# llehouerou/go-mp3

Hardware: AMD Instinct MI355X
Metric: MP3 frames/sec (44.1 kHz stereo 128 kbps) at 1/2/4/8 GPUs; max |ΔPCM| LSB (higher is better)
Workload: dtype f32; 1 GPU; c3: 1,024 independently seeded streams x 1,024 frames, 44.1 kHz stereo 128 kbps CBR (synthetic Layer III writer, seeds 1..1024); streams_per_gpu=1024, mode=fast (+-1 LSB vs reference), parallelism=1 independent ranks (stream sharding, no data-path collective), granules_per_gpu=2097152, chunks=16384, halo_granules=30720

## Files before the change

go-mp3_amd/csrc/granule_fast.hip:

```cpp
#pragma clang fp contract(fast)
#include <type_traits>

#include "dct32.h"
#include "dct4_18.h"
#include "xlane.h"

namespace mp3g {
namespace v3 {
#ifndef MP3G_FAST_PRIO
#define MP3G_FAST_PRIO 1
#endif
#ifndef MP3G_FAST_WG_WAVES
#define MP3G_FAST_WG_WAVES 8
#endif
constexpr int kWaves = MP3G_FAST_WG_WAVES;
namespace {

using common::hdr_combo;
using common::hdr_mode;
using common::hdr_nch;
__device__ __forceinline__ int pcm_sample(float sum) {
  return (int)__builtin_amdgcn_fmed3f(sum * 32767.0f, -32767.0f, 32767.0f);
}

constexpr int kLanes = 64;
using pk::f2;
__device__ __forceinline__ f2 pfma(f2 a, f2 b, f2 c) { return __builtin_elementwise_fma(a, b, c); }
__device__ __forceinline__ f2 bcast(float v) { return (f2){v, v}; }
__device__ __forceinline__ int kPretab(int sfb) { return (int)((0x2fe95400000ull >> (2 * sfb)) & 3u); }
constexpr int kHist = 16;
#ifndef MP3G_FAST_WAVES_PER_SIMD
#define MP3G_FAST_WAVES_PER_SIMD 4
#endif
constexpr int kSlots = kHist + 18;
static_assert(kSlots == kFastRingSlots, "FastTables::sinfo indexes the staged ring");
#ifndef MP3G_FAST_DWIN_STRIDE
#define MP3G_FAST_DWIN_STRIDE 20
#endif
constexpr int kDwinStride = MP3G_FAST_DWIN_STRIDE;

struct __align__(16) SharedSmem {
  float4 winp[4][2][9];
  float isr[8][2];
  float dwin[32][kDwinStride];
  uint2 lbd[kCombos][32];
  __device__ uint32_t lband_at(int c, int k) const { return lbd[c][k].x; }
  float p43[kFastP43];
};
struct __align__(16) WaveSmem {
  float ring[2][32][kSlots];
  mp3g_granule desc;
  _Float16 expo[2 * 22 + 2 * 39];
  __device__ float* expo_gain() { return reinterpret_cast<float*>(expo); }
  __device__ const float* expo_gain() const { return reinterpret_cast<const float*>(expo); }
  uint32_t zone[8][2];
};
constexpr uint32_t kZones = 8;
static_assert(kZones <= kZoneListPerChunk, "zone list smaller than a chunk's zones");

__device__ __forceinline__ void load_lines(const int16_t* coef, uint32_t g, int lane, uint32_t cw[9],
                                           int nbytes = (int)(MP3G_COEF_PER_GRANULE * sizeof(int16_t))) {
  const __amdgpu_buffer_rsrc_t rc = __builtin_amdgcn_make_buffer_rsrc(
      const_cast<int16_t*>(coef + (size_t)g * MP3G_COEF_PER_GRANULE), (short)0, nbytes,
      0x00020000);
  const int off = (lane >> 5) * 1152 + (lane & 31) * 36;
#pragma unroll
  for (int i = 0; i < 3; i++) {
    const auto v = __builtin_amdgcn_raw_buffer_load_b96(rc, off + 12 * i, 0, 0);
    cw[3 * i] = v[0];
    cw[3 * i + 1] = v[1];
    cw[3 * i + 2] = v[2];
  }
}

__device__ __forceinline__ void load_lines_lim(const int16_t* coef, uint32_t g, int lane, uint32_t cw[9], int nbytes,
                                               int lim) {
  const __amdgpu_buffer_rsrc_t rc = __builtin_amdgcn_make_buffer_rsrc(
      const_cast<int16_t*>(coef + (size_t)g * MP3G_COEF_PER_GRANULE), (short)0, nbytes,
      0x00020000);
  const int l0 = 18 * (lane & 31);
  const int off = (lane >> 5) * 1152 + 2 * l0;
#pragma unroll
  for (int i = 0; i < 3; i++) {
    const auto v = __builtin_amdgcn_raw_buffer_load_b96(rc, l0 + 6 * i < lim ? off + 12 * i : kNoRecord, 0, 0);
    cw[3 * i] = v[0];
    cw[3 * i + 1] = v[1];
    cw[3 * i + 2] = v[2];
  }
}
__device__ __forceinline__ uint32_t load_desc_dword(const mp3g_granule* gran, uint32_t g, int lane, bool valid) {
  const __amdgpu_buffer_rsrc_t rd = __builtin_amdgcn_make_buffer_rsrc(
      const_cast<mp3g_granule*>(gran + g), (short)0, valid ? (int)sizeof(mp3g_granule) : 0, 0x00020000);
  return __builtin_amdgcn_raw_buffer_load_b32(rd, 4 * lane, 0, 0);
}
__device__ __forceinline__ uint32_t desc_word(uint32_t dv, int k) {
  return (uint32_t)__builtin_amdgcn_readlane((int)dv, k);
}
__device__ __forceinline__ uint32_t desc_byte(uint32_t dv, int b) {
  return ((uint32_t)__builtin_amdgcn_ds_bpermute((b >> 2) << 2, (int)dv) >> (8 * (b & 3))) & 0xffu;
}
static_assert(sizeof(mp3g_granule) == 160 && offsetof(mp3g_granule, ch) == 8 && sizeof(mp3g_channel) == 72 &&
                  offsetof(mp3g_channel, scalefac_l) == 11,
              "descriptor dword layout");

__device__ __forceinline__ int count1_lim(const mp3g_granule* gran, uint32_t g, int lane) {
  const uint32_t h = gran[g].header;
  const int c0 = gran[g].ch[0].count1, c1 = gran[g].ch[1].count1;
  return (lane >> 5) ? (common::hdr_nch(h) == 2 ? c1 : 0) : c0;
}

__device__ void prologue(const ChunkDesc& cd, const mp3g_granule* gran, uint64_t* w_out, int init_in[2],
                         int lane) {
  const uint64_t c0 = cd.out_first, s0 = cd.stream_first;
  const bool have_in = cd.flags & kChunkStateIn;
  if (c0 == s0) {
    *w_out = c0;
    init_in[0] = init_in[1] = have_in;
    return;
  }
  const uint64_t start0 = (c0 >= 2 && c0 - 2 > s0) ? c0 - 2 : s0;
  const bool st1 = hdr_nch(gran[c0 - 1].header) == 2;
  const bool st2 = (c0 >= 2 && c0 - 2 >= s0) ? hdr_nch(gran[c0 - 2].header) == 2 : false;
  if (st1 && st2) {
    *w_out = start0;
    init_in[0] = init_in[1] = (start0 == s0) && have_in;
    return;
  }
  int any = 0;
  for (uint32_t k = lane; k < cd.n_out; k += kLanes) any |= hdr_nch(gran[c0 + k].header) == 2;
  const bool need1 = __ballot(any) != 0 || (cd.flags & kChunkStateOut);
  uint64_t start1 = c0;
  bool ch1_from_in = false;
  if (need1) {
    int found = 0;
    uint64_t p2 = 0;
    for (uint64_t hi = c0; hi > s0 && found < 2;) {
      const uint64_t lo = hi - s0 > kLanes ? hi - kLanes : s0;
      const uint64_t g = hi - 1 - lane;
      const bool stereo = ((uint64_t)lane < hi - lo) && hdr_nch(gran[g].header) == 2;
      uint64_t m = __ballot(stereo);
      while (m && found < 2) {
        const int b = __ffsll((unsigned long long)m) - 1;
        found++;
        if (found == 2) p2 = hi - 1 - b;
        m &= m - 1;
      }
      hi = lo;
    }
    if (found == 2) start1 = p2;
    else if (found == 1) start1 = s0;
    else ch1_from_in = true;
  }
  const uint64_t w = start0 < start1 ? start0 : start1;
  *w_out = w;
  init_in[0] = (w == s0) && have_in;
  init_in[1] = ch1_from_in ? have_in : ((w == s0) && have_in);
}

__device__ __forceinline__ void wave_sync() {
  __builtin_amdgcn_fence(__ATOMIC_RELEASE, "wavefront");
  __builtin_amdgcn_wave_barrier();
  __builtin_amdgcn_fence(__ATOMIC_ACQUIRE, "wavefront");
}

__device__ __forceinline__ void settle_vmem() { __builtin_amdgcn_s_waitcnt(0x0f70); }

__device__ __forceinline__ float self(bool c, float a, float b) {
  const int m = -(int)c;
  return __int_as_float((__float_as_int(a) & m) | (__float_as_int(b) & ~m));
}
__device__ __forceinline__ int seli(bool c, int a, int b) {
  const int m = -(int)c;
  return (a & m) | (b & ~m);
}

__device__ __forceinline__ float requant_fast(int xi, _Float16 e) {
  const float xf = (float)xi;
  const float t = __builtin_fmaf(__builtin_amdgcn_logf(fabsf(xf)), 1.0f / 3.0f, (float)e);
  return xf * __builtin_amdgcn_exp2f(t);
}

__device__ __forceinline__ float requant_gain(uint32_t xw, float g) {
  const float xf = (float)(int16_t)xw;
  return xf * __builtin_amdgcn_exp2f(__builtin_amdgcn_logf(fabsf(xf)) * (1.0f / 3.0f)) * g;
}

__device__ __forceinline__ float x_from_v(const float* v, int m) { return m >= 16 ? v[m - 16] : -v[48 - m]; }
template <int kS = kSlots>
__device__ __forceinline__ float v_from_x(const float* x, int i) {
  if (i < 16) return x[kS * dct32::kPosOfM[16 + i]];
  if (i == 16) return 0.0f;
  if (i < 48) return -x[kS * dct32::kPosOfM[48 - i]];
  return -x[kS * dct32::kPosOfM[i - 48]];
}

#ifndef MP3G_HOT_S
#define MP3G_HOT_S 4.0f
#endif
constexpr float kHotS = MP3G_HOT_S;
#ifndef MP3G_HOT_CHECK
#define MP3G_HOT_CHECK 1
#endif
#ifndef MP3G_HOT_L1
#define MP3G_HOT_L1 64.0f
#endif
constexpr float kHotL1 = MP3G_HOT_L1;

__device__ __forceinline__ float rmul(float a, float b) {
#pragma clang fp contract(off)
  return a * b;
}
__device__ __forceinline__ float radd(float a, float b) {
#pragma clang fp contract(off)
  return a + b;
}
__device__ __forceinline__ float rsub(float a, float b) {
#pragma clang fp contract(off)
  return a - b;
}

__device__ __forceinline__ float requant_exact(int xi, _Float16 e) {
  const int n4 = (int)((float)e * 4.0f);
  const float v = __builtin_ldexpf(g_req[n4 & 3][min(abs(xi), 8206)], n4 >> 2);
  return xi < 0 ? -v : v;
}

__device__ __forceinline__ const float* vtab(const float* p) {
  asm volatile("" : "+s"(p));
  return p;
}
typedef const float __attribute__((address_space(4))) cfloat4;
__device__ __forceinline__ cfloat4* stab(const float* p) {
  cfloat4* q = (cfloat4*)p;
  asm volatile("" : "+s"(q));
  return q;
}

template <int kS = kSlots>
__device__ __forceinline__ bool slot_sums_hot(const float (&ring)[2][32][kS], int nch, int cur = kHist) {
  const int lane = lane_fresh();
  const int c = lane >> 5, slot = lane & 31;
  float sum = 0.0f;
  if (c < nch && slot < 18) {
#pragma unroll
    for (int sb = 0; sb < 32; sb++) sum += fabsf(ring[c][sb][cur + slot]);
  }
  return __builtin_amdgcn_ballot_w64(sum > kHotL1) != 0;
}

__device__ __forceinline__ float max_abs18(const float* v) {
  float m = 0.0f;
#pragma unroll
  for (int j = 0; j < 18; j++) m = fmaxf(m, fabsf(v[j]));
  return m;
}

__device__ __forceinline__ void imdct_exact(const float x[18], int bt, int k, bool act, f2 stp[9], float o[18]) {
#pragma clang fp contract(off)
  const float sodd = (k & 1) ? -1.0f : 1.0f;
  const float* c12 = vtab(&g_fast.cos12[0][0]);
  const float* c36 = vtab(&g_fast.c36[0][0]);
  const float* win = vtab(&g_fast.win[0][0]) + 36 * bt;
  float st[18];
#pragma unroll
  for (int q = 0; q < 9; q++) {
    st[q] = stp[q].x;
    st[17 - q] = stp[q].y;
  }
  if (bt == 2) {
#pragma unroll
    for (int pos = 0; pos < 36; pos++) {
      float raw = 0.0f;
#pragma unroll
      for (int wi = 0; wi < 3; wi++) {
        const int p = pos - 6 - 6 * wi;
        if (p < 0 || p >= 12) continue;
        float sum = 0.0f;
#pragma unroll
        for (int m = 0; m < 6; m++) sum = sum + x[wi + 3 * m] * c12[12 * m + p];
        raw = raw + sum * win[p];
      }
      const float f = (pos & 1) ? raw * sodd : raw;
      if (pos < 18) o[pos] = f + st[pos];
      else if (act) st[pos - 18] = f;
    }
  } else {
    float d[18];
#pragma unroll
    for (int q = 0; q < 18; q++) {
      float s = 0.0f;
#pragma unroll
      for (int m = 0; m < 18; m++) s = s + x[m] * c36[18 * m + q];
      d[q] = s;
    }
#pragma unroll
    for (int pos = 0; pos < 36; pos++) {
      const float v = pos < 9 ? d[pos] : pos < 18 ? -d[17 - pos] : pos < 27 ? d[pos - 9] : d[44 - pos];
      const float raw = v * win[pos];
      const float f = (pos & 1) ? raw * sodd : raw;
      if (pos < 18) o[pos] = f + st[pos];
      else if (act) st[pos - 18] = f;
    }
  }
#pragma unroll
  for (int q = 0; q < 9; q++) stp[q] = (f2){st[q], st[17 - q]};
}

template <int kS = kSlots>
__device__ __forceinline__ void matrix_exact(float* colu) {
#pragma clang fp contract(off)
  float S[32];
#pragma unroll
  for (int j = 0; j < 32; j++) S[j] = colu[kS * j];
  for (int m = 0; m < 32; m++) {
    const float* row = vtab(&g_fast.nrow[m][0]);
    float s = 0.0f;
#pragma unroll
    for (int j = 0; j < 32; j++) s = s + row[j] * S[j];
    colu[kS * dct32::kPosOfM[m]] = s;
  }
}

template <int cur = kHist>
__device__ __forceinline__ void window_exact(const float* RA, const float* RB, int k, f2 acc2[9]) {
#pragma clang fp contract(off)
  float dw[16];
#pragma unroll
  for (int j = 0; j < 16; j++) dw[j] = vtab(&g_fast.dwin[0][0])[16 * k + j];
#pragma unroll
  for (int ss = 0; ss < 18; ss++) {
    float sum = 0.0f;
#pragma unroll
    for (int j = 0; j < 16; j++) sum = sum + ((j & 1) ? RB : RA)[cur + ss - j] * dw[j];
    const float t = sum * 32767.0f;
    if (ss & 1) acc2[ss >> 1].y = t;
    else acc2[ss >> 1].x = t;
  }
}
// ... 161 lines not shown
    } else {
      const __amdgpu_buffer_rsrc_t rl = __builtin_amdgcn_make_buffer_rsrc(
          const_cast<uint32_t*>(&g_fast.linfo[P.combo][0]), (short)0, 576 * 4, 0x00020000);
#pragma unroll
      for (int j = 0; j < 18; j++) {
        const uint32_t info = __builtin_amdgcn_raw_buffer_load_b32(rl, 4 * (18 * k0 + j), 0, 0);
        const int sfl = info & 31, sfs = (info >> 5) & 15, wown = (info >> 11) & 3;
        const bool lp = mixed0 && sfl < 8 && sfl >= nl_is;
        const bool sp = sfs < 12 && (!mixed0 || sfs >= 3) && sfs >= ns_is;
        const int pl = lp ? min((int)C0.scalefac_l[min(sfl, 21)], 7) : 7;
        const int ps = sp ? min((int)C0.scalefac_s[min(sfs, 12)][min(wown, 2)], 7) : 7;
        x[j] = x[j] * sh.isr[pl][ch] * sh.isr[ps][ch];
      }
    }
  }
}

template <bool kExact>
__device__ __forceinline__ void antialias_stage(float x[18], const GranParams& P, bool act, int k) {
  const bool sw = P.shortblk;
  const bool skip = !act || (sw && !P.mixed);
  const int sblim = (sw && P.mixed) ? 2 : 32;
  const bool lower = !skip && k >= 1 && k < sblim;
  const bool upper = !skip && k < 31 && k + 1 < sblim;
  float up[8], dn[8];
#pragma unroll
  for (int i = 0; i < 8; i++) {
    up[i] = xl::from_prev(x[17 - i]);
    dn[i] = xl::from_next(x[i]);
  }
#pragma unroll
  for (int i = 0; i < 8; i++) {
    const float cs = g_fast.aa_cs[i], ca = g_fast.aa_ca[i];
    const float ui = x[i], li = x[17 - i];
    if (kExact) {
      x[i] = self(lower, radd(rmul(ui, cs), rmul(up[i], ca)), ui);
      x[17 - i] = self(upper, rsub(rmul(li, cs), rmul(dn[i], ca)), li);
    } else {
      x[i] = self(lower, ui * cs + up[i] * ca, ui);
      x[17 - i] = self(upper, li * cs - dn[i] * ca, li);
    }
  }
}

__device__ __forceinline__ int imdct_block_type(uint32_t d1, int k) {
  int bt = (int)((d1 >> 16) & 3u);
  if ((d1 & 0xff00ff00u) == 0x01000100u && k < 2) bt = 0;
  return bt;
}

__device__ __forceinline__ void imdct_fast(const float x[18], int bt, int nch, bool act, float sodd,
                                           const SharedSmem& sh, f2 stp[9], float o[18]) {
  if (bt == 2) {
    float st[18];
#pragma unroll
    for (int q = 0; q < 9; q++) {
      st[q] = stp[q].x;
      st[17 - q] = stp[q].y;
    }
#pragma unroll
    for (int pos = 0; pos < 36; pos++) {
      float raw = 0.0f;
#pragma unroll
      for (int wi = 0; wi < 3; wi++) {
        const int p = pos - 6 - 6 * wi;
        if (p < 0 || p >= 12) continue;
        float sum = 0.0f;
#pragma unroll
        for (int m = 0; m < 6; m++) sum += x[wi + 3 * m] * dct4::kCos12[p][m];
        raw += sum * dct4::kWin12[p];
      }
      if (pos & 1) raw *= sodd;
      if (pos < 18) o[pos] = raw + st[pos];
      else st[pos - 18] = self(act, raw, st[pos - 18]);
    }
#pragma unroll
    for (int q = 0; q < 9; q++) stp[q] = (f2){st[q], st[17 - q]};
  } else {
    f2 P[9];
    dct4::dct4_18_pk(x, P);
    const float4* Wq = sh.winp[bt][lane_fresh() & 1];
    auto overlap = [&](auto frozen) {
#pragma unroll
      for (int kk = 0; kk < 9; kk++) {
        const int q = kk <= 4 ? 8 - 2 * kk : 2 * kk - 9;
        const float za = kk <= 4 ? P[kk].y : P[kk].x;
        const float zb = kk <= 4 ? P[kk].x : P[kk].y;
        const float4 w = Wq[q];
        const f2 oq = pfma(bcast(za), (f2){w.x, w.y}, stp[q]);
        o[q] = oq.x;
        o[17 - q] = oq.y;
        const f2 ns = bcast(zb) * (f2){w.z, w.w};
        if constexpr (decltype(frozen)::value)
          stp[q] = (f2){self(act, ns.x, stp[q].x), self(act, ns.y, stp[q].y)};
        else
          stp[q] = ns;
      }
    };
    if (nch == 2) overlap(std::false_type{});
    else overlap(std::true_type{});
  }
}

__device__ __forceinline__ void init_state(WaveSmem& s, const mp3g_state* sin, const int init_in[2], int lane,
                                           f2 stp[9]) {
  const int ch = lane >> 5, k = lane & 31;
  const float sodd = (k & 1) ? -1.0f : 1.0f;
  const bool in0 = init_in[0] && sin, in1 = init_in[1] && sin;
  const bool from_in = ch ? in1 : in0;
#pragma unroll
  for (int q = 0; q < 9; q++) {
    const float a = from_in ? sin->store[ch][k][q] : 0.0f, b = from_in ? sin->store[ch][k][17 - q] : 0.0f;
    stp[q] = (f2){(q & 1) ? a * sodd : a, (q & 1) ? b : b * sodd};
  }
  for (int e = lane; e < 2 * 15 * 32; e += kLanes) {
    const int c = e / (15 * 32), blk = (e >> 5) % 15, m = e & 31;
    const bool in = c ? in1 : in0;
    s.ring[c][dct32::kPosOfM[m]][kHist - 1 - blk] = in ? x_from_v(&sin->vvec[c][64 * blk], m) : 0.0f;
  }
}

__device__ __forceinline__ void load_granule(const mp3g_granule* gran, const int16_t* coef, uint32_t g, int lane,
                                             WaveSmem& s, uint32_t cw[9]) {
  load_lines_lim(coef, g, lane, cw, (int)(MP3G_COEF_PER_GRANULE * sizeof(int16_t)), count1_lim(gran, g, lane));
  if (lane < 10) reinterpret_cast<uint4*>(&s.desc)[lane] = reinterpret_cast<const uint4*>(gran + g)[lane];
}

__device__ __forceinline__ bool replay_needs_v(const mp3g_granule* gran, uint32_t g, uint32_t out_from) {
  if (g >= out_from || g + 1 >= out_from) return true;
  return hdr_nch(gran[g + 1].header) < hdr_nch(gran[g].header);
}

__device__ __forceinline__ bool exact_granule(const mp3g_granule* __restrict__ gran, const int16_t* __restrict__ coef,
                                              int16_t* __restrict__ pcm, WaveSmem& s, const SharedSmem& sh,
                                              uint32_t g, bool out, bool need_v, f2 stp[9]) {
  const int lane = lane_fresh();
  const int ch = lane >> 5, k = lane & 31, hi = lane >> 5;
  uint32_t cw[9];
  load_granule(gran, coef, g, lane, s, cw);
  wave_sync();
  const GranParams P = granule_params(s, ch);
  const bool act = ch < P.nch;
  float x[18];
  front_gather<true>(x, cw, s, P, ch, k);
  stereo_stage(x, s, sh, P, ch);
  antialias_stage<true>(x, P, act, k);
  float o[18];
  imdct_exact(x, imdct_block_type(P.d1, k), k, act, stp, o);
  const bool hot1 = __builtin_amdgcn_ballot_w64((act ? max_abs18(o) : 0.0f) > kHotS) != 0;
  if (act) {
#pragma unroll
    for (int j = 0; j < 18; j++) s.ring[ch][k][kHist + j] = o[j];
  }
  wave_sync();
  const bool hot = hot1 && slot_sums_hot(s.ring, P.nch);
  if (need_v && act && (lane & 31) < 18) matrix_exact(&s.ring[ch][0][kHist + (lane & 31)]);
  wave_sync();
  uint32_t pk[9] = {};
  if (out) {
    const int pa = dct32::kPosOfM[k < 16 ? 16 + k : (k == 16 ? 0 : 48 - k)];
    const int pb = dct32::kPosOfM[k < 16 ? 16 - k : k - 16];
    f2 acc2[9];
    window_exact(&s.ring[ch][pa][0], &s.ring[ch][pb][0], k, acc2);
    pack_pcm(acc2, P.nch, pk);
  }
  store_pcm(pcm, g, out, pk, hi, k);
  wave_sync();
  if (ch < P.nch && need_v) {
    f2* col = reinterpret_cast<f2*>(&s.ring[ch][k][0]);
#pragma unroll
    for (int q = 0; q < 8; q++) col[q] = col[9 + q];
  }
  wave_sync();
  return hot;
}

__device__ __forceinline__ uint32_t zone_end(const mp3g_granule* __restrict__ gran, uint32_t g, uint32_t end) {
  uint32_t e = g + 2;
  if (hdr_nch(__builtin_amdgcn_readfirstlane(gran[g].header)) == 2) {
    uint32_t n = g + 1;
    while (n < end && hdr_nch(__builtin_amdgcn_readfirstlane(gran[n].header)) == 1) n++;
    if (n + 1 > e) e = n + 1;
  }
  return e < end ? e : end;
}

template <class Smem>
__device__ __forceinline__ void record_hot(Smem& s, uint32_t& nz, const mp3g_granule* __restrict__ gran, uint32_t g,
                                           uint32_t out_first, uint32_t end) {
  const uint32_t zs = g > out_first ? g : out_first;
  const uint32_t ze = zone_end(gran, g, end);
  if (zs >= ze) return;
  const uint32_t last_end = nz ? __builtin_amdgcn_readfirstlane(s.zone[nz - 1][1]) : 0u;
  if (nz > 0 && zs <= last_end) {
    s.zone[nz - 1][1] = ze > last_end ? ze : last_end;
  } else if (nz < kZones) {
    s.zone[nz][0] = zs;
    s.zone[nz][1] = ze;
    nz = __builtin_amdgcn_readfirstlane(nz + 1);
  } else {
    s.zone[kZones - 1][1] = end;
  }
  wave_sync();
}

}

constexpr int kPhases = 8;
template <bool kStamp, bool kHotCount = false, int kFmt = (int)MP3G_OUT_S16>
__global__ void __launch_bounds__(kLanes * kWaves, MP3G_FAST_WAVES_PER_SIMD)
granule_fast_kernel(const ChunkDesc* __restrict__ chunks, uint32_t n_chunks, const mp3g_granule* __restrict__ gran,
                    const int16_t* __restrict__ coef, const mp3g_state* __restrict__ state_in,
                    mp3g_state* __restrict__ state_out, int16_t* __restrict__ pcm,
                    void* __restrict__ aux_arg) {
  unsigned long long* const stamps = kStamp ? static_cast<unsigned long long*>(aux_arg) : nullptr;
  uint32_t* const aux = kStamp ? nullptr : static_cast<uint32_t*>(aux_arg);
  unsigned long long ph[kPhases] = {}, tprev = 0, rt[4] = {};
  if constexpr (kStamp) rt[0] = __builtin_amdgcn_s_memrealtime();
  auto stamp = [&](int p) {
    if constexpr (kStamp) {
      const unsigned long long t = __builtin_amdgcn_s_memtime();
      ph[p] += t - tprev;
      tprev = t;
    }
  };
  __shared__ struct {
    SharedSmem sh;
    WaveSmem w[kWaves];
  } lds;
  SharedSmem& sh = lds.sh;
  WaveSmem* const wsm = lds.w;
  auto shared_init = [&]() {
    const int t = threadIdx.x;
    for (int e = t; e < 4 * 2 * 9; e += kLanes * kWaves) {
      const int bt = e / 18, par = (e / 9) & 1, q = e % 9;
      const float* W = g_fast.win[bt];
      const float sq = par && (q & 1) ? -1.0f : 1.0f, sr = par && !(q & 1) ? -1.0f : 1.0f;
      sh.winp[bt][par][q] = make_float4(W[q] * sq, -W[17 - q] * sr, -W[18 + q] * sq, -W[35 - q] * sr);
    }
    for (int e = t; e < 16; e += kLanes * kWaves) (&sh.isr[0][0])[e] = e < 14 ? (&g_fast.is_ratio[0][0])[e] : 1.0f;
    for (int e = t; e < 32 * 16; e += kLanes * kWaves) sh.dwin[e >> 4][e & 15] = (&g_fast.dwin[0][0])[e] * 32767.0f;
    for (int e = t; e < kCombos * 32; e += kLanes * kWaves) {
      const uint32_t lb = (&g_fast.lband[0][0])[e];
      uint32_t d = 0;
      for (int i = 1; i <= 8; i++) d |= ((lb >> (5 + 2 * i)) & 1u) * (15u << (4 * (i - 1)));
      (&sh.lbd[0][0])[e] = make_uint2(lb, d);
    }
    for (int e = t; e < kFastP43; e += kLanes * kWaves) sh.p43[e] = g_fast.p43[e];
  };
  const int lane = threadIdx.x & (kLanes - 1);
  const uint32_t ci = __builtin_amdgcn_readfirstlane(blockIdx.x * kWaves + (threadIdx.x >> 6));
  if (ci >= n_chunks) {
    shared_init();
    __syncthreads();
    return;
  }
  WaveSmem& s = wsm[threadIdx.x >> 6];
  const ChunkDesc cd = chunks[ci];
  const int ch = lane >> 5, k = lane & 31;
  const int pa = dct32::kPosOfM[k < 16 ? 16 + k : (k == 16 ? 0 : 48 - k)];
  const int pb = dct32::kPosOfM[k < 16 ? 16 - k : k - 16];

  uint64_t w64;
  int init_in[2];
  prologue(cd, gran, &w64, init_in, lane);
  const uint32_t w = __builtin_amdgcn_readfirstlane((uint32_t)w64);
  const uint32_t out_first = __builtin_amdgcn_readfirstlane((uint32_t)cd.out_first);
  const uint32_t end = __builtin_amdgcn_readfirstlane((uint32_t)(cd.out_first + cd.n_out));
  const mp3g_state* sin = state_in ? state_in + cd.stream : nullptr;
  WinGeom wgeom = {nullptr, 0u, 0u, 0u};
  if constexpr (fmt_is_windowed(kFmt)) wgeom = win_geom(pcm, state_out, cd.stream);

  const float sodd = (k & 1) ? -1.0f : 1.0f;
  f2 stp[9];
  {
    const bool in0 = init_in[0] && sin, in1 = init_in[1] && sin;
    const bool from_in = ch ? in1 : in0;
#pragma unroll
    for (int q = 0; q < 9; q++) {
      const float a = from_in ? sin->store[ch][k][q] : 0.0f, b = from_in ? sin->store[ch][k][17 - q] : 0.0f;
      stp[q] = (f2){(q & 1) ? a * sodd : a, (q & 1) ? b : b * sodd};
    }
    for (int e = lane; e < 2 * 15 * 32; e += kLanes) {
      const int c = e / (15 * 32), blk = (e >> 5) % 15, m = e & 31;
      const bool in = c ? in1 : in0;
      s.ring[c][dct32::kPosOfM[m]][kHist - 1 - blk] = in ? x_from_v(&sin->vvec[c][64 * blk], m) : 0.0f;
    }
  }

  uint32_t cw[9] = {};
  uint32_t dv = 0, dvn = 0;
  if (w < end) {
    load_lines_lim(coef, w, lane, cw, (int)(MP3G_COEF_PER_GRANULE * sizeof(int16_t)), count1_lim(gran, w, lane));
    dv = load_desc_dword(gran, w, lane, true);
    dvn = load_desc_dword(gran, w + 1, lane, w + 1 < end);
  }
  shared_init();
  settle_vmem();
  __syncthreads();

  uint32_t pk[9] = {};
  const int hi = lane >> 5;

  auto window_acc = [&](f2 (&acc2)[9]) {
    float dw[16];
    {
      const float4* d4 = reinterpret_cast<const float4*>(&sh.dwin[k][0]);
#pragma unroll
      for (int q = 0; q < 4; q++) {
        const float4 v = d4[q];
        dw[4 * q] = v.x;
        dw[4 * q + 1] = v.y;
        dw[4 * q + 2] = v.z;
        dw[4 * q + 3] = v.w;
      }
    }
    const f2* RA = reinterpret_cast<const f2*>(&s.ring[ch][pa][0]);
    const float* RB = &s.ring[ch][pb][0];
#pragma unroll
    for (int p = 0; p < 9; p++) acc2[p] = bcast(0.0f);
#pragma unroll
    for (int v = -14; v <= 16; v += 2) {
      const f2 A = RA[(kHist + v) / 2];
      const f2 B = {RB[kHist + v - 1], RB[kHist + v]};
#pragma unroll
      for (int t = 0; t < 8; t++) {
        const int p = v / 2 + t;
        if (p >= 0 && p < 9) {
          acc2[p] = pfma(bcast(dw[2 * t]), A, acc2[p]);
          acc2[p] = pfma(bcast(dw[2 * t + 1]), B, acc2[p]);
        }
      }
    }
  };
  StreamGeom geom = {0u, 0u};
  if constexpr (kFmt == (int)MP3G_OUT_F32_PLANAR)
    geom = StreamGeom{(uint32_t)__builtin_amdgcn_readfirstlane((uint32_t)cd.stream_first),
                      (uint32_t)__builtin_amdgcn_readfirstlane(cd.stream_n)};
  auto window_store = [&](uint32_t g, bool out, int nch) {
    if constexpr (kFmt != (int)MP3G_OUT_S16) {
      typename PcmRegs<kFmt>::type pr;
      if (out) {
        f2 acc2[9];
        window_acc(acc2);
        pack_granule<kFmt>(acc2, nch, pr);
      } else {
#pragma unroll
        for (int i = 0; i < (int)(sizeof(pr) / sizeof(pr[0])); i++) pr[i] = 0;
      }
      store_granule<kFmt>(pcm, geom, wgeom, g, out, pr);
      return;
    }
    if (out) {
      f2 acc2[9];
      window_acc(acc2);
      pack_pcm(acc2, nch, pk);
    }
    {
      const __amdgpu_buffer_rsrc_t rp = __builtin_amdgcn_make_buffer_rsrc(
          pcm + (size_t)g * 1152, (short)0, out ? MP3G_PCM_BYTES_PER_GRANULE : 0, 0x00020000);
#pragma unroll
      for (int p = 0; p < 9; p++)
        __builtin_amdgcn_raw_buffer_store_b32(pk[p], rp, 4 * (32 * (2 * p + hi) + k), 0, 2);
    }
  };

  if constexpr (kStamp) {
    tprev = __builtin_amdgcn_s_memtime();
    rt[1] = __builtin_amdgcn_s_memrealtime();
  }
  const uint32_t span = end - w, span2 = 2 * span, span3 = 3 * span;
  uint32_t nz = 0;
  uint32_t n_flagged = 0;
  const uint32_t t3 = end - (span3 >> 2), t2 = end - (span2 >> 2), t1 = end - (span >> 2);
  if (MP3G_FAST_PRIO) __builtin_amdgcn_s_setprio(3);
  for (uint32_t g = w; g < end; g++) {
    if (MP3G_FAST_PRIO) {
      if (g == t1) __builtin_amdgcn_s_setprio(0);
      else if (g == t2) __builtin_amdgcn_s_setprio(1);
      else if (g == t3) __builtin_amdgcn_s_setprio(2);
    }
    const bool out = g >= out_first;
    const uint32_t h = desc_word(dv, 0);
    bool need_v = true;
    if (!out && g + 1 < out_first) need_v = hdr_nch(gran[g + 1].header) < hdr_nch(h);
    const int nch = hdr_nch(h), combo = hdr_combo(h);
    const bool act = ch < nch;
    const uint32_t cp0[2] = {desc_word(dv, 2), desc_word(dv, 20)};
    const uint32_t cp1[2] = {desc_word(dv, 3), desc_word(dv, 21)};
    auto is_short = [](uint32_t d1) { return (d1 & 0x00ffff00u) == 0x00020100u; };
    const bool all_long = !is_short(cp1[0]) && (nch == 1 || !is_short(cp1[1]));
    if (!all_long || (nch == 2 && hdr_mode(h) == 1 && (h & 0x10u))) {
      const int l = lane_fresh();
      if (l < 40) reinterpret_cast<uint32_t*>(&s.desc)[l] = dv;
      wave_sync();
    }
    const uint32_t d0 = (act && ch) ? cp0[1] : cp0[0], d1 = (act && ch) ? cp1[1] : cp1[0];

    {
      const int e = lane_fresh();
      const int sfl_byte = (int)desc_byte(dv, 19 + 72 * ch + (e & 31));
      if ((e & 31) < 22) {
        const int sfb = e & 31;
        const int v = (int)((d0 >> 16) & 0xffu) - 210 -
                      ((d0 >> 24) ? 4 : 2) * (sfl_byte + (int)(d1 & 0xffu) * kPretab(sfb));
        if (all_long) s.expo_gain()[22 * ch + sfb] = __builtin_amdgcn_exp2f(0.25f * (float)v);
        else s.expo[22 * ch + sfb] = (_Float16)(0.25f * (float)v);
      }
      if (!all_long) {
        for (int r0 = e; r0 < 2 * 39; r0 += kLanes) {
          const int c = r0 >= 39, r = r0 - 39 * c, sfb = r / 3, win = r - 3 * sfb;
          const uint32_t a0 = c ? cp0[1] : cp0[0];
          const mp3g_channel& D = s.desc.ch[c];
          const int v = (int)((a0 >> 16) & 0xffu) - 210 - 8 * (int)D.subblock_gain[win] -
                        ((a0 >> 24) ? 4 : 2) * (int)D.scalefac_s[sfb][win];
          s.expo[44 + r0] = (_Float16)(0.25f * (float)v);
        }
      }
    }
    const int count1 = (int)(d0 & 0xffffu);
    const bool shortblk = is_short(d1);
    const bool mixed = (d1 >> 24) != 0;
    wave_sync();
    stamp(0);

    float x[18];
    if (all_long) {
      const int kl = lane_fresh() & 31;
      const uint2 lbd = sh.lbd[combo][kl];
      const uint32_t lb = lbd.x, d4 = lbd.y;
      const char* eb = reinterpret_cast<const char*>(&s.expo_gain()[22 * ch + (int)(lb & 31u)]);
      float gq[9];
#pragma unroll
      for (int q = 0; q < 9; q++)
        gq[q] = *reinterpret_cast<const float*>(eb + __builtin_popcount(d4 & (q == 8 ? ~0u : (1u << (4 * q)) - 1u)));
      const char* tb = reinterpret_cast<const char*>(&sh.p43[0]);
      uint32_t big = 0;
#pragma unroll
      for (int q = 0; q < 9; q++) {
        uint32_t t;
        asm("v_pk_mad_u16 %0, %1, 4, %2 op_sel_hi:[1,0,1]" : "=v"(t) : "v"(cw[q]), "s"(0x00010001u * 2u * kFastP43));
        big |= t;
        x[2 * q] = *reinterpret_cast<const float*>(tb + (t & 0xffffu));
        x[2 * q + 1] = *reinterpret_cast<const float*>(tb + (t >> 16));
      }
#pragma unroll
      for (int j = 0; j < 18; j++) x[j] *= gq[j >> 1];
      if (big & (0x00010001u * (0x10000u - 4u * kFastP43))) {
#pragma unroll
        for (int q = 0; q < 9; q++) {
          x[2 * q] = requant_gain(cw[q] & 0xffffu, gq[q]);
          x[2 * q + 1] = requant_gain(cw[q] >> 16, gq[q]);
        }
      }
    } else {
      int nsfs = 0;
#pragma unroll
      for (int b = 0; b < 13; b++) nsfs += 3 * (int)g_fast.sfb_short[combo][b] < count1;
      {
        uint32_t* col = reinterpret_cast<uint32_t*>(&s.ring[ch][k][kHist]);
#pragma unroll
        for (int q = 0; q < 9; q++) col[q] = cw[q];
      }
      wave_sync();
      const int16_t* rch = reinterpret_cast<const int16_t*>(&s.ring[ch][0][kHist]);
      auto plain = [&](uint32_t d) { return is_short(d) && !(d >> 24); };
      const bool plain_short = plain(cp1[0]) && (nch == 1 || plain(cp1[1]));
      const __amdgpu_buffer_rsrc_t rl = __builtin_amdgcn_make_buffer_rsrc(
          const_cast<uint32_t*>(plain_short ? &g_fast.sinfo[combo][0] : &g_fast.linfo[combo][0]), (short)0,
          576 * 4, 0x00020000);
      const int L0 = 18 * (lane_fresh() & 31);
      uint32_t infw[18];
#pragma unroll
      for (int q = 0; q < 9; q++) {
        const auto v = __builtin_amdgcn_raw_buffer_load_b64(rl, 4 * L0 + 8 * q, 0, 0);
        infw[2 * q] = v[0];
        infw[2 * q + 1] = v[1];
      }
      if (plain_short) {
        const int ebase = 44 + 39 * ch;
#pragma unroll
        for (int j = 0; j < 18; j++) {
          const uint32_t inf = infw[j];
          const int sfs = inf & 15u;
          const bool started = sfs < nsfs;
          const bool reord = sfs == 0 || started;
          const int xi = rch[seli(reord, (int)(inf >> 16), 2 * kSlots * (lane_fresh() & 31) + j)];
          const int e = seli(reord, (int)((inf >> 4) & 63u), (int)((inf >> 10) & 63u));
          x[j] = self(started, requant_fast(xi, s.expo[ebase + e]), (float)xi);
        }
      } else {
#pragma unroll
        for (int j = 0; j < 18; j++) {
          const int L = L0 + j;
          const uint32_t inf = infw[j];
          const int sfl = inf & 31, sfs = (inf >> 5) & 15, wsrc = (inf >> 9) & 3, wown = (inf >> 11) & 3;
          const int srcr = inf >> 13;
          const bool longlike = !shortblk || (mixed && L < 36);
          const bool started = sfs < nsfs;
          const bool reord = sfs == (mixed ? 3 : 0) || started;
          const int src = seli(longlike || !reord, L, srcr);
          const int win = seli(reord, wsrc, wown);
          const int eidx = seli(longlike, 22 * ch + sfl, 44 + 39 * ch + 3 * sfs + win);
          const bool process = longlike ? (shortblk || L < count1) : started;
          const int sk = (src * 3641) >> 16;
          const int xi = rch[2 * kSlots * sk + (src - 18 * sk)];
          x[j] = self(process, requant_fast(xi, s.expo[eidx]), (float)xi);
        }
      }
      wave_sync();
    }
    stamp(1);
    if (nch == 2 && hdr_mode(h) == 1 && (h & 0x30u)) {
      const mp3g_channel& C0 = s.desc.ch[0];
      const int c1r = (int)(cp0[1] & 0xffffu);
      const int msmax = max((int)(cp0[0] & 0xffffu), c1r);
      const bool ms = h & 0x20u, is = h & 0x10u;
      const bool short0 = is_short(cp1[0]);
      const bool mixed0 = (cp1[0] >> 24) != 0;
      const float inv_sqrt2 = 0.70710678118654752440f;
      if (ms) {
        auto ms_pair = [&](float& u, float& v) {
          const auto r = __builtin_amdgcn_permlane32_swap(__float_as_int(u), __float_as_int(v), false, false);
          const float a = __int_as_float(r[0]), b = __int_as_float(r[1]);
          const f2 pq = (f2){a + b, a - b} * bcast(inv_sqrt2);
          const auto r2 = __builtin_amdgcn_permlane32_swap(__float_as_int(pq.x), __float_as_int(pq.y), false, false);
          u = __int_as_float(r2[0]);
          v = __int_as_float(r2[1]);
        };
        if (all_long && !is) {
#pragma unroll
          for (int j = 0; j < 18; j += 2) ms_pair(x[j], x[j + 1]);
        } else {
          const int left = msmax - 18 * (lane_fresh() & 31);
#pragma unroll
          for (int j = 0; j < 18; j += 2) {
            float n0 = x[j], n1 = x[j + 1];
            ms_pair(n0, n1);
            x[j] = j < left ? n0 : x[j];
            x[j + 1] = j + 1 < left ? n1 : x[j + 1];
          }
        }
      }
      if (is) {
        const int k0 = lane_fresh() & 31;
        int nl_is = 0, ns_is = 0;
#pragma unroll
        for (int b = 0; b < 23; b++) nl_is += (int)g_fast.sfb_long[combo][b] < c1r;
#pragma unroll
        for (int b = 0; b < 14; b++) ns_is += 3 * (int)g_fast.sfb_short[combo][b] < c1r;
        if (!short0) {
          const uint32_t lb = sh.lbd[combo][k0].x;
#pragma unroll
          for (int j = 0; j < 18; j++) {
            const int sfl = (int)(lb & 31u) + __builtin_popcount((lb >> 5) & ((2u << j) - 1u));
            const int pos = min((int)C0.scalefac_l[min(sfl, 21)], 7);
            const float rr = sh.isr[pos][ch];
            x[j] = (sfl < 21 && sfl >= nl_is) ? x[j] * rr : x[j];
          }
        } else {
          const __amdgpu_buffer_rsrc_t rl = __builtin_amdgcn_make_buffer_rsrc(
              const_cast<uint32_t*>(&g_fast.linfo[combo][0]), (short)0, 576 * 4, 0x00020000);
          uint32_t infw[18];
#pragma unroll
          for (int q = 0; q < 9; q++) {
            const auto v = __builtin_amdgcn_raw_buffer_load_b64(rl, 4 * 18 * k0 + 8 * q, 0, 0);
            infw[2 * q] = v[0];
            infw[2 * q + 1] = v[1];
          }
#pragma unroll
          for (int j = 0; j < 18; j++) {
            const uint32_t info = infw[j];
            const int sfl = info & 31, sfs = (info >> 5) & 15, wown = (info >> 11) & 3;
            const bool lp = mixed0 && sfl < 8 && sfl >= nl_is;
            const bool sp = sfs < 12 && (!mixed0 || sfs >= 3) && sfs >= ns_is;
            const int pl = lp ? min((int)C0.scalefac_l[min(sfl, 21)], 7) : 7;
            const int ps = sp ? min((int)C0.scalefac_s[min(sfs, 12)][min(wown, 2)], 7) : 7;
            x[j] = x[j] * sh.isr[pl][ch] * sh.isr[ps][ch];
          }
        }
      }
    }
    {
      const bool sw = shortblk;
      const bool skip = !act || (sw && !mixed);
      const int sblim = (sw && mixed) ? 2 : 32;
      const bool lower = !skip && k >= 1 && k < sblim;
      const bool upper = !skip && k < 31 && k + 1 < sblim;
      float up[8], dn[8];
#pragma unroll
      for (int i = 0; i < 8; i++) {
        up[i] = xl::from_prev(x[17 - i]);
        dn[i] = xl::from_next(x[i]);
      }
#pragma unroll
      for (int i = 0; i < 8; i++) {
        const float cs = g_fast.aa_cs[i], ca = g_fast.aa_ca[i];
        const float ui = x[i], li = x[17 - i];
        x[i] = self(lower, ui * cs + up[i] * ca, ui);
        x[17 - i] = self(upper, li * cs - dn[i] * ca, li);
      }
    }

    stamp(2);
    float o[18];
    {
      int bt = (int)((d1 >> 16) & 3u);
      if ((d1 & 0xff00ff00u) == 0x01000100u && k < 2) bt = 0;
      if (bt == 2) {
        float st[18];
#pragma unroll
        for (int q = 0; q < 9; q++) {
          st[q] = stp[q].x;
          st[17 - q] = stp[q].y;
        }
#pragma unroll
        for (int pos = 0; pos < 36; pos++) {
          float raw = 0.0f;
#pragma unroll
          for (int wi = 0; wi < 3; wi++) {
            const int p = pos - 6 - 6 * wi;
            if (p < 0 || p >= 12) continue;
            float sum = 0.0f;
#pragma unroll
            for (int m = 0; m < 6; m++) sum += x[wi + 3 * m] * dct4::kCos12[p][m];
            raw += sum * dct4::kWin12[p];
          }
          if (pos & 1) raw *= sodd;
          if (pos < 18) o[pos] = raw + st[pos];
          else st[pos - 18] = self(act, raw, st[pos - 18]);
        }
#pragma unroll
        for (int q = 0; q < 9; q++) stp[q] = (f2){st[q], st[17 - q]};
      } else {
        f2 P[9];
        dct4::dct4_18_pk(x, P);
        const float4* Wq = sh.winp[bt][lane_fresh() & 1];
        auto overlap = [&](auto frozen) {
#pragma unroll
          for (int kk = 0; kk < 9; kk++) {
            const int q = kk <= 4 ? 8 - 2 * kk : 2 * kk - 9;
            const float za = kk <= 4 ? P[kk].y : P[kk].x;
            const float zb = kk <= 4 ? P[kk].x : P[kk].y;
            const float4 w = Wq[q];
            const f2 oq = pfma(bcast(za), (f2){w.x, w.y}, stp[q]);
            o[q] = oq.x;
            o[17 - q] = oq.y;
            const f2 ns = bcast(zb) * (f2){w.z, w.w};
            if constexpr (decltype(frozen)::value)
              stp[q] = (f2){self(act, ns.x, stp[q].x), self(act, ns.y, stp[q].y)};
            else
              stp[q] = ns;
          }
        };
        if (nch == 2) overlap(std::false_type{});
        else overlap(std::true_type{});
      }
    }
#if MP3G_HOT_CHECK
    const bool hot1 = __builtin_amdgcn_ballot_w64((act ? max_abs18(o) : 0.0f) > kHotS) != 0;
#endif
    stamp(3);
    const bool more = g + 1 < end;
    uint32_t pdw;
    {
      {
        const uint32_t nh = desc_word(dvn, 0);
        const int c0 = (int)(desc_word(dvn, 2) & 0xffffu);
        const int c1 = (int)(desc_word(dvn, 20) & 0xffffu);
        const int lim = ch ? (hdr_nch(nh) == 2 ? c1 : 0) : c0;
        load_lines_lim(coef, g + 1, lane, cw, more ? (int)(MP3G_COEF_PER_GRANULE * sizeof(int16_t)) : 0, lim);
      }
      pdw = load_desc_dword(gran, g + 2, lane_fresh(), g + 2 < end);
    }

    if (need_v && act) {
#pragma unroll
      for (int j = 0; j < 18; j++) s.ring[ch][k][kHist + j] = o[j];
    }
    wave_sync();
#if MP3G_HOT_CHECK
    if (hot1 && need_v && slot_sums_hot(s.ring, nch)) {
      record_hot(s, nz, gran, g, out_first, end);
      if constexpr (kHotCount) n_flagged++;
    }
#endif
    stamp(4);
    {
      const int slot = lane & 31;
      if (need_v && act && slot < 18) {
        float* colu = &s.ring[ch][0][kHist + slot];
        dct32::f2 sp[16];
#pragma unroll
        for (int q = 0; q < 16; q++) sp[q] = (dct32::f2){colu[kSlots * 2 * q], colu[kSlots * (2 * q + 1)]};
        dct32::dct2_32_to(sp, [&](int t, dct32::f2 v) {
          colu[kSlots * dct32::kColX[t]] = v.x;
          colu[kSlots * dct32::kColY[t]] = v.y;
        });
      }
    }
    stamp(5);
    wave_sync();

    dv = dvn;
    dvn = pdw;

    window_store(g, out, nch);
    wave_sync();
    stamp(6);

    if (ch < nch && need_v) {
      f2* col = reinterpret_cast<f2*>(&s.ring[ch][k][0]);
#pragma unroll
      for (int q = 0; q < 8; q++) col[q] = col[9 + q];
    }
    wave_sync();
    stamp(7);
  }
  if constexpr (kStamp) rt[2] = __builtin_amdgcn_s_memrealtime();

  auto export_state = [&](const f2 (&st)[9]) {
    if (!(cd.flags & kChunkStateOut)) return;
    mp3g_state* so = state_out + cd.stream;
    const int c = lane_fresh() >> 5, kk = lane_fresh() & 31;
    const float sg = (kk & 1) ? -1.0f : 1.0f;
#pragma unroll
    for (int q = 0; q < 9; q++) {
      so->store[c][kk][q] = (q & 1) ? st[q].x * sg : st[q].x;
      so->store[c][kk][17 - q] = (q & 1) ? st[q].y : st[q].y * sg;
    }
    for (int e = lane_fresh(); e < 2 * 1024; e += kLanes) {
      const int cc = e >> 10, blk = (e >> 6) & 15, i = e & 63;
      so->vvec[cc][64 * blk + i] = blk < 15 ? v_from_x(&s.ring[cc][0][kHist - 1 - blk], i) : 0.0f;
    }
  };
  export_state(stp);

  uint32_t* const hot_count = aux ? aux + 4 : nullptr;
  if (!kStamp && nz) {
    uint32_t* const zone_count = aux;
    ChunkDesc* const zone_list = reinterpret_cast<ChunkDesc*>(aux + 8);
    const uint32_t zone_cap = __builtin_amdgcn_readfirstlane(aux[2]);
    uint32_t n_pieces = 0;
    for (uint32_t i = 0; i < nz; i++) {
      const uint32_t zs = __builtin_amdgcn_readfirstlane(s.zone[i][0]), ze = __builtin_amdgcn_readfirstlane(s.zone[i][1]);
      n_pieces += (ze - zs + kZonePiece - 1) / kZonePiece;
    }
    uint32_t base = 0;
    if (lane_fresh() == 0) base = atomicAdd(zone_count, n_pieces);
    base = __builtin_amdgcn_readfirstlane(base);
    for (uint32_t i = 0; i < nz; i++) {
      const uint32_t zs = __builtin_amdgcn_readfirstlane(s.zone[i][0]), ze = __builtin_amdgcn_readfirstlane(s.zone[i][1]);
      const uint32_t np = (ze - zs + kZonePiece - 1) / kZonePiece;
      const uint32_t l = (uint32_t)lane_fresh();
      if (l < np && base + l < zone_cap) {
        const uint32_t ps = zs + l * kZonePiece, pe = min(ps + kZonePiece, ze);
        ChunkDesc z;
        z.out_first = ps;
        z.stream_first = cd.stream_first;
        z.n_out = pe - ps;
        z.stream = cd.stream;
        z.flags = (cd.flags & kChunkStateIn) | (pe == end ? (cd.flags & kChunkStateOut) : 0u);
        z.stream_n = kFmt == (int)MP3G_OUT_F32_PLANAR ? cd.stream_n : 0u;
        zone_list[base + l] = z;
      }
      base += np;
    }
  }
  if constexpr (!kStamp && kHotCount) {
    if (nz || n_flagged) {
      uint32_t n_out = 0;
      for (uint32_t i = 0; i < nz; i++)
        n_out += __builtin_amdgcn_readfirstlane(s.zone[i][1]) - __builtin_amdgcn_readfirstlane(s.zone[i][0]);
      if (lane_fresh() == 0) {
        atomicAdd(hot_count + 0, n_out);
        atomicAdd(hot_count + 1, nz);
        atomicAdd(hot_count + 2, n_flagged);
      }
    }
  }
  if (kStamp && nz) {
    f2 zst[9];
    uint32_t done = 0;
    bool have = false;
    uint32_t n_out = 0, n_run = 0;
    for (uint32_t i = 0; i < nz; i++) {
      const uint32_t zs = __builtin_amdgcn_readfirstlane(s.zone[i][0]);
      uint32_t ze = __builtin_amdgcn_readfirstlane(s.zone[i][1]);
      if (have && ze <= done) continue;
      uint32_t gz = done;
      if (!have || zs > done) {
        ChunkDesc cr = cd;
        cr.out_first = zs;
        cr.n_out = end - zs;
        uint64_t wz;
        int zin[2];
        prologue(cr, gran, &wz, zin, lane_fresh());
        init_state(s, sin, zin, lane_fresh(), zst);
        gz = __builtin_amdgcn_readfirstlane((uint32_t)wz);
        have = true;
      }
      for (; gz < ze; gz++) {
        const bool nv = replay_needs_v(gran, gz, zs);
        n_run++;
        n_out += gz >= zs ? 1u : 0u;
        if (exact_granule(gran, coef, pcm, s, sh, gz, gz >= zs, nv, zst)) {
          const uint32_t e = zone_end(gran, gz, end);
          ze = e > ze ? e : ze;
        }
      }
      done = gz;
    }
    if (done >= end) export_state(zst);
    if (kHotCount && hot_count && lane_fresh() == 0) {
      atomicAdd(hot_count + 0, n_out);
      atomicAdd(hot_count + 1, nz);
      atomicAdd(hot_count + 2, n_flagged);
      atomicAdd(hot_count + 3, n_run);
    }
  }
  if constexpr (kStamp) {
    rt[3] = __builtin_amdgcn_s_memrealtime();
    if (lane == 0) {
      for (int p = 0; p < kPhases; p++) stamps[(size_t)ci * kFastStampSlots + p] = ph[p];
      for (int p = 0; p < 4; p++) stamps[(size_t)ci * kFastStampSlots + kPhases + p] = rt[p];
    }
  }
}

}
}
```

Before: 281.2 million frames/s.

## Replace per-granule ring history shift with ping-pong layout parity

Instead of copying 16 history slots down the ring after every granule, the ring now alternates between two physical layouts chosen by a parity bit. Window accumulation, the DCT writes and the spectrum staging translate virtual slots through region-based offsets. This removes the LDS copy and one wave_sync per granule. The cost is extra addressing logic, some split non-pairable loads, and special handling for mono frames and state export; one settle_vmem is also added.

```diff
diff --git a/go-mp3_amd/csrc/granule_fast.hip b/go-mp3_amd/csrc/granule_fast.hip
--- a/go-mp3_amd/csrc/granule_fast.hip
+++ b/go-mp3_amd/csrc/granule_fast.hip
@@ -34,6 +34,52 @@
 #endif
 constexpr int kSlots = kHist + 18;
 static_assert(kSlots == kFastRingSlots, "FastTables::sinfo indexes the staged ring");
+__device__ __forceinline__ constexpr int rphys(int P, int z) { return !P ? z : z <= 15 ? 18 + z : z <= 18 ? z : z - 18; }
+__device__ __forceinline__ constexpr int rregion(int z) { return z <= 15 ? 0 : z <= 18 ? 1 : 2; }
+__device__ __forceinline__ constexpr int rshift(int P, int z) { return rregion(z) == 0 ? 18 * P : rregion(z) == 2 ? -18 * P : 0; }
+__device__ __forceinline__ constexpr int rcur(int P) { return P ? 1 : kHist; }
+namespace ring_map {
+constexpr bool bijective(int P) {
+  unsigned long long seen = 0;
+  for (int z = 1; z <= 33; z++) {
+    const int p = rphys(P, z);
+    if (p < 1 || p > 33 || ((seen >> p) & 1)) return false;
+    seen |= 1ull << p;
+  }
+  return true;
+}
+constexpr bool hands_over(int P) {
+  for (int z = 1; z <= 15; z++)
+    if (rphys(P, 18 + z) != rphys(!P, z)) return false;
+  return true;
+}
+constexpr bool cur_contiguous(int P) {
+  for (int j = 0; j < 18; j++)
+    if (rphys(P, 16 + j) < rcur(P) || rphys(P, 16 + j) >= rcur(P) + 18) return false;
+  return true;
+}
+constexpr bool a_pairs_aligned(int P) {
+  for (int v = -14; v <= 16; v += 2) {
+    const int a = rphys(P, 16 + v), b = rphys(P, 17 + v);
+    if (P && v == 2) {
+      if (a != 18 || b != 1) return false;
+    } else if ((a & 1) || b != a + 1) {
+      return false;
+    }
+  }
+  return true;
+}
+constexpr bool shifts_agree(int P) {
+  for (int z = 1; z <= 33; z++)
+    if (rphys(P, z) != z + rshift(P, z)) return false;
+  return true;
+}
+static_assert(shifts_agree(0) && shifts_agree(1), "rshift is rphys as a displacement");
+static_assert(bijective(0) && bijective(1), "a layout maps the virtual slots 1..33 onto the positions 1..33");
+static_assert(hands_over(0) && hands_over(1), "the history changes layout without moving");
+static_assert(cur_contiguous(0) && cur_contiguous(1), "rcur: the written positions");
+static_assert(a_pairs_aligned(0) && a_pairs_aligned(1), "8-B aligned A pairs");
+}
 #ifndef MP3G_FAST_DWIN_STRIDE
 #define MP3G_FAST_DWIN_STRIDE 20
 #endif
@@ -801,7 +847,7 @@
   uint32_t pk[9] = {};
   const int hi = lane >> 5;
 
-  auto window_acc = [&](f2 (&acc2)[9]) {
+  auto window_acc = [&](uint32_t par, f2 (&acc2)[9]) {
     float dw[16];
     {
       const float4* d4 = reinterpret_cast<const float4*>(&sh.dwin[k][0]);
@@ -814,14 +860,19 @@
         dw[4 * q + 3] = v.w;
       }
     }
-    const f2* RA = reinterpret_cast<const f2*>(&s.ring[ch][pa][0]);
+    const float* RA = &s.ring[ch][pa][0];
     const float* RB = &s.ring[ch][pb][0];
+    const int d = par ? 18 : 0;
+    const float* const RAr[3] = {RA + d, RA, RA - d};
+    const float* const RBr[3] = {RB + d, RB, RB - d};
 #pragma unroll
     for (int p = 0; p < 9; p++) acc2[p] = bcast(0.0f);
 #pragma unroll
     for (int v = -14; v <= 16; v += 2) {
-      const f2 A = RA[(kHist + v) / 2];
-      const f2 B = {RB[kHist + v - 1], RB[kHist + v]};
+      const int za = kHist + v, zb = kHist + v - 1;
+      const f2 A = rregion(za) == rregion(za + 1) ? *reinterpret_cast<const f2*>(RAr[rregion(za)] + za)
+                                                  : (f2){RAr[rregion(za)][za], RAr[rregion(za + 1)][za + 1]};
+      const f2 B = {RBr[rregion(zb)][zb], RBr[rregion(zb + 1)][zb + 1]};
 #pragma unroll
       for (int t = 0; t < 8; t++) {
         const int p = v / 2 + t;
@@ -836,12 +887,12 @@
   if constexpr (kFmt == (int)MP3G_OUT_F32_PLANAR)
     geom = StreamGeom{(uint32_t)__builtin_amdgcn_readfirstlane((uint32_t)cd.stream_first),
                       (uint32_t)__builtin_amdgcn_readfirstlane(cd.stream_n)};
-  auto window_store = [&](uint32_t g, bool out, int nch) {
+  auto window_store = [&](uint32_t g, bool out, int nch, uint32_t par) {
     if constexpr (kFmt != (int)MP3G_OUT_S16) {
       typename PcmRegs<kFmt>::type pr;
       if (out) {
         f2 acc2[9];
-        window_acc(acc2);
+        window_acc(par, acc2);
         pack_granule<kFmt>(acc2, nch, pr);
       } else {
 #pragma unroll
@@ -852,7 +903,7 @@
     }
     if (out) {
       f2 acc2[9];
-      window_acc(acc2);
+      window_acc(par, acc2);
       pack_pcm(acc2, nch, pk);
     }
     {
@@ -873,7 +924,10 @@
   uint32_t n_flagged = 0;
   const uint32_t t3 = end - (span3 >> 2), t2 = end - (span2 >> 2), t1 = end - (span >> 2);
   if (MP3G_FAST_PRIO) __builtin_amdgcn_s_setprio(3);
+  uint32_t lay = 0;
   for (uint32_t g = w; g < end; g++) {
+    const uint32_t par = lay & 1u;
+    const int cur = par ? rcur(1) : rcur(0);
     if (MP3G_FAST_PRIO) {
       if (g == t1) __builtin_amdgcn_s_setprio(0);
       else if (g == t2) __builtin_amdgcn_s_setprio(1);
@@ -956,13 +1010,13 @@
       int nsfs = 0;
 #pragma unroll
       for (int b = 0; b < 13; b++) nsfs += 3 * (int)g_fast.sfb_short[combo][b] < count1;
-      {
-        uint32_t* col = reinterpret_cast<uint32_t*>(&s.ring[ch][k][kHist]);
+      if (act) {
+        uint32_t* col = reinterpret_cast<uint32_t*>(&s.ring[ch][k][0]) + cur;
 #pragma unroll
         for (int q = 0; q < 9; q++) col[q] = cw[q];
       }
       wave_sync();
-      const int16_t* rch = reinterpret_cast<const int16_t*>(&s.ring[ch][0][kHist]);
+      const int16_t* rch = reinterpret_cast<const int16_t*>(&s.ring[ch][0][0] + cur);
       auto plain = [&](uint32_t d) { return is_short(d) && !(d >> 24); };
       const bool plain_short = plain(cp1[0]) && (nch == 1 || plain(cp1[1]));
       const __amdgpu_buffer_rsrc_t rl = __builtin_amdgcn_make_buffer_rsrc(
@@ -1007,6 +1061,7 @@
           x[j] = self(process, requant_fast(xi, s.expo[eidx]), (float)xi);
         }
       }
+      settle_vmem();
       wave_sync();
     }
     stamp(1);
@@ -1174,12 +1229,22 @@
     }
 
     if (need_v && act) {
-#pragma unroll
-      for (int j = 0; j < 18; j++) s.ring[ch][k][kHist + j] = o[j];
+      float* col = &s.ring[ch][k][0];
+      float* const colr[3] = {nullptr, col, col - (par ? 18 : 0)};
+#pragma unroll
+      for (int j = 0; j < 18; j += 2) {
+        const int z = kHist + j;
+        if (rregion(z) == rregion(z + 1)) {
+          *reinterpret_cast<f2*>(colr[rregion(z)] + z) = (f2){o[j], o[j + 1]};
+        } else {
+          colr[rregion(z)][z] = o[j];
+          colr[rregion(z + 1)][z + 1] = o[j + 1];
+        }
+      }
     }
     wave_sync();
 #if MP3G_HOT_CHECK
-    if (hot1 && need_v && slot_sums_hot(s.ring, nch)) {
+    if (hot1 && need_v && slot_sums_hot(s.ring, nch, cur)) {
       record_hot(s, nz, gran, g, out_first, end);
       if constexpr (kHotCount) n_flagged++;
     }
@@ -1188,7 +1253,7 @@
     {
       const int slot = lane & 31;
       if (need_v && act && slot < 18) {
-        float* colu = &s.ring[ch][0][kHist + slot];
+        float* colu = &s.ring[ch][0][0] + cur + slot;
         dct32::f2 sp[16];
 #pragma unroll
         for (int q = 0; q < 16; q++) sp[q] = (dct32::f2){colu[kSlots * 2 * q], colu[kSlots * (2 * q + 1)]};
@@ -1204,21 +1269,33 @@
     dv = dvn;
     dvn = pdw;
 
-    window_store(g, out, nch);
+    window_store(g, out, nch, par);
     wave_sync();
     stamp(6);
 
-    if (ch < nch && need_v) {
-      f2* col = reinterpret_cast<f2*>(&s.ring[ch][k][0]);
-#pragma unroll
-      for (int q = 0; q < 8; q++) col[q] = col[9 + q];
-    }
-    wave_sync();
+    if (nch == 2) {
+      lay = need_v ? par ^ 1u : par;
+    } else if (need_v) {
+      if (!(lay & 2u)) {
+        if (ch == 1) {
+          f2* col2 = reinterpret_cast<f2*>(&s.ring[1][k][0]);
+          if (par) {
+#pragma unroll
+            for (int q = 0; q < 8; q++) col2[q] = col2[9 + q];
+          } else {
+#pragma unroll
+            for (int q = 0; q < 8; q++) col2[9 + q] = col2[q];
+          }
+        }
+        wave_sync();
+      }
+      lay = (par ^ 1u) | 2u;
+    }
     stamp(7);
   }
   if constexpr (kStamp) rt[2] = __builtin_amdgcn_s_memrealtime();
 
-  auto export_state = [&](const f2 (&st)[9]) {
+  auto export_state = [&](const f2 (&st)[9], uint32_t Pn) {
     if (!(cd.flags & kChunkStateOut)) return;
     mp3g_state* so = state_out + cd.stream;
     const int c = lane_fresh() >> 5, kk = lane_fresh() & 31;
@@ -1230,10 +1307,12 @@
     }
     for (int e = lane_fresh(); e < 2 * 1024; e += kLanes) {
       const int cc = e >> 10, blk = (e >> 6) & 15, i = e & 63;
-      so->vvec[cc][64 * blk + i] = blk < 15 ? v_from_x(&s.ring[cc][0][kHist - 1 - blk], i) : 0.0f;
+      const int z = kHist - 1 - blk;
+      so->vvec[cc][64 * blk + i] = blk < 15 ? v_from_x(&s.ring[cc][0][0] + (Pn ? 18 + z : z), i) : 0.0f;
     }
   };
-  export_state(stp);
+  static_assert(rphys(1, 1) == 19 && rphys(1, 15) == 33 && rphys(0, 15) == 15, "export_state's history positions");
+  export_state(stp, lay & 1u);
 
   uint32_t* const hot_count = aux ? aux + 4 : nullptr;
   if (!kStamp && nz) {
@@ -1310,7 +1389,7 @@
       }
       done = gz;
     }
-    if (done >= end) export_state(zst);
+    if (done >= end) export_state(zst, 0u);
     if (kHotCount && hot_count && lane_fresh() == 0) {
       atomicAdd(hot_count + 0, n_out);
       atomicAdd(hot_count + 1, nz);
```

Measured after the change: 286.9 million frames/s, median of 6. +2.0%, better.
